# rewaifu/resselt

Hardware: AMD Instinct MI355X
Metric: output megapixels/sec, RealESRGAN-x4plus 1080p→4K, 1/2/4/8 MI355X (higher is better)
Workload: dtype fp16; 1 GPU; RealESRGAN-x4plus (RRDBNet nf64 nb23 gc32 x4), 1x3x1080x1920 fp32 frame per GPU -> 1x3x4320x7680, residual-dense-block convolutions (92 % of the MACs) in ONE fp16 product on hi planes, conv_first / upsampling / HR / last convolutions in three bf16 products on split planes, trunk convolution in three fp16 products; f32 accumulate, synthetic uniform(+-1/sqrt(fan_in)) weights; precision=auto -> mixed, io=fp32 [N,C,H,W] tensors in and out, tile_parallel=single tile

## Files before the change

include/resselt_amd.h:

```cpp
#ifndef RESSELT_AMD_H
#define RESSELT_AMD_H

#include <stdint.h>

#ifdef __cplusplus
extern "C" {
#endif

#define RSA_VERSION 400

#define RSA_OK 0
#define RSA_E_ARG (-1)
#define RSA_E_UNSUPPORTED (-2)
#define RSA_E_ALIGN (-3)
#define RSA_E_FP16_RANGE (-5)
#define RSA_E_INTERNAL (-4)

enum rsa_act {
  RSA_ACT_NONE = 0,
  RSA_ACT_LRELU = 1,
  RSA_ACT_MISH = 2,
  RSA_ACT_SILU = 3,
  RSA_ACT_GELU = 4,
  RSA_ACT_SPAB_GATE = 5,
// ... 57 lines not shown
  int32_t tile_order;
  int32_t lo8_flags;
  int32_t reserved_lo8;
  int64_t lo8_batch_stride;
} rsa_conv_params;
#define RSA_LO8_RES1 1
#define RSA_LO8_RES2 2
#define RSA_LO8_OUT 4

int rsa_conv2d(const rsa_conv_params* p, void* stream);
int rsa_conv2d_list(const rsa_conv_params* list, int32_t n, void* stream);

int rsa_conv2d_pair(const rsa_conv_params* a, const rsa_conv_params* b, void* stream);
int rsa_conv_pair_fusable(const rsa_conv_params* a, const rsa_conv_params* b);

int rsa_check_status(void);

int rsa_check_finite(const void* data, int32_t dtype, int64_t count, void* stream);

int64_t rsa_packed_weight_bytes(int32_t cout, int32_t cin_planes, int32_t ksize, int32_t products);
int64_t rsa_packed_weight_bytes_layout(int32_t cout, int32_t cin_planes, int32_t ksize, int32_t products, int32_t layout);

int rsa_conv_cout_tiles(int32_t cout);

int rsa_conv_weight_layout(const rsa_conv_params* p);
int rsa_pack_weights(const float* w_oihw, int32_t cout, int32_t cin, int32_t cin_planes, int32_t ksize, int32_t products, int32_t layout,
                     int32_t fmt, void* out, void* stream);

const char* rsa_conv_kernel_name(const rsa_conv_params* p);

int rsa_debug_ring_aborts(void);
int rsa_debug_set_ring_spin_limit(int32_t polls);
int rsa_debug_set_ring(int32_t mode);
int rsa_debug_set_pair(int32_t mode);

int rsa_nchw_to_planes(const void* x, int32_t dtype, int32_t batch, int32_t C, int32_t H, int32_t W, int32_t src_h, int32_t src_w,
                       int32_t unshuffle, const float* mean, float scale, void* out_hi, void* out_lo, int64_t out_plane_stride,
                       int64_t out_batch_stride, int32_t out_fmt, void* stream);

int rsa_planes_to_nchw(const void* hi, const void* lo, int64_t plane_stride, int64_t batch_stride, int32_t batch,
                       int32_t C, int32_t H, int32_t W, int32_t fmt, float* out, void* stream);

typedef struct rsa_dysample_params {
  int32_t batch;
  int32_t H, W;
  int32_t C;
  int32_t groups;
  int32_t scale;
  int32_t out_ch;
  const float* x_f32;
  const float* offscope;
  const float* init_pos;
  const float* end_w;
  const float* end_b;
  void* out_nchw;
  int32_t out_dtype;
} rsa_dysample_params;

int rsa_dysample(const rsa_dysample_params* p, void* stream);

typedef struct rsa_layernorm_params {
  int32_t batch;
  int32_t H, W;
  int32_t C;
  float eps;
  const float* x_f32;
// ... 716 lines not shown
```

resselt_amd/csrc/capi.hip:

```cpp
#include <hip/hip_runtime.h>
#include <stdint.h>
#include <stdio.h>
#include <string.h>

#include <type_traits>

#include "common.h"
#include "resselt_amd.h"

namespace rsa {

static thread_local char g_err[256] = "";

int set_error(int code, const char* msg) {
  if (code > 0)
    snprintf(g_err, sizeof(g_err), "%s (hipError %d: %s)", msg, code, hipGetErrorString((hipError_t)code));
  else
    snprintf(g_err, sizeof(g_err), "%s", msg);
  return code;
}

typedef __attribute__((ext_vector_type(8))) __bf16 bf16x8;

template <typename T>
// ... 218 lines not shown
  if (word == nullptr) return rsa::set_error(RSA_E_INTERNAL, "check_finite: no host-visible status word (pinned allocation failed)");
  const int64_t vecs = count / (dtype == RSA_F32 ? 4 : 8);
  const unsigned grid = rsa::grid_for(vecs > 0 ? vecs : 1, 256 * 4);
  if (dtype == RSA_F32)
    hipLaunchKernelGGL(rsa::check_finite_kernel<float>, dim3(grid), dim3(256), 0, (hipStream_t)stream, (const float*)data, count, word);
  else if (dtype == RSA_F16)
    hipLaunchKernelGGL(rsa::check_finite_kernel<_Float16>, dim3(grid), dim3(256), 0, (hipStream_t)stream, (const _Float16*)data, count, word);
  else if (dtype == RSA_BF16)
    hipLaunchKernelGGL(rsa::check_finite_kernel<__bf16>, dim3(grid), dim3(256), 0, (hipStream_t)stream, (const __bf16*)data, count, word);
  else
    return rsa::set_error(RSA_E_ARG, "check_finite: dtype must be RSA_F32, RSA_F16 or RSA_BF16");
  const int rc = (int)hipGetLastError();
  return rc ? rsa::set_error(rc, "check_finite: launch failed") : RSA_OK;
}

int rsa_conv_cout_tiles(int32_t cout) { return rsa::conv_nct(cout); }

int rsa_conv_weight_layout(const rsa_conv_params* p) {
  if (p == nullptr) return rsa::set_error(RSA_E_ARG, "rsa_conv_weight_layout: null params");
  return rsa::conv_weight_layout(*p);
}

const char* rsa_conv_kernel_name(const rsa_conv_params* p) { return p == nullptr ? "" : rsa::conv_kernel_name(*p); }

int rsa_debug_ring_aborts(void) { return (int)rsa::conv_ring_aborts(); }

int rsa_check_status(void) { return rsa::conv_check_status(); }

int rsa_debug_set_ring_spin_limit(int32_t polls) {
  rsa::conv_set_ring_spin_limit(polls);
  return RSA_OK;
}

int rsa_debug_set_ring(int32_t mode) {
  rsa::conv_ring_override(mode);
  return RSA_OK;
}

int64_t rsa_packed_weight_bytes(int32_t cout, int32_t cin_planes, int32_t ksize, int32_t products) {
  if (cout < 1 || cin_planes < 1 || (ksize != 1 && ksize != 3) || (products != 1 && products != 3)) return RSA_E_ARG;
  const int64_t ct = (cout + 15) / 16;
  const int64_t chunks = (cin_planes + 3) / 4;
  const int64_t nhl = products == 3 ? 2 : 1;
  return chunks * ksize * ksize * ct * nhl * 64 * 16;
}

int rsa_nchw_to_planes(const void* x, int32_t dtype, int32_t batch, int32_t C, int32_t H, int32_t W, int32_t src_h, int32_t src_w,
                       int32_t unshuffle, const float* mean, float scale, void* out_hi, void* out_lo, int64_t out_plane_stride,
                       int64_t out_batch_stride, int32_t out_fmt, void* stream) {
  if (out_fmt != RSA_PF_BF16 && out_fmt != RSA_PF_F16) return rsa::set_error(RSA_E_ARG, "nchw_to_planes: out_fmt must be an rsa_plane_fmt");
  if (unshuffle < 1) return rsa::set_error(RSA_E_ARG, "nchw_to_planes: unshuffle must be >= 1");
  if (x == nullptr || out_hi == nullptr || batch < 1 || C < 1 || H < 1 || W < 1) return rsa::set_error(RSA_E_ARG, "nchw_to_planes: bad argument");
  {
    const int64_t fh = (int64_t)H * unshuffle, fw = (int64_t)W * unshuffle;
    if (src_h < 1 || src_w < 1 || src_h > fh || src_w > fw || fh - src_h >= src_h || fw - src_w >= src_w)
      return rsa::set_error(RSA_E_ARG, "nchw_to_planes: source size must satisfy src <= plane size * unshuffle < 2*src (reflect padding)");
  }
  if (dtype < RSA_F32 || dtype > RSA_U8) return rsa::set_error(RSA_E_ARG, "nchw_to_planes: bad dtype");
  if (((uintptr_t)out_hi | (uintptr_t)out_lo) & 15) return rsa::set_error(RSA_E_ALIGN, "nchw_to_planes: outputs must be 16-byte aligned");
  const int64_t total = (int64_t)batch * ((C * unshuffle * unshuffle + 7) / 8) * H * W;
  hipLaunchKernelGGL(rsa::nchw_to_planes_kernel, dim3(rsa::grid_for(total, 256)), dim3(256), 0, (hipStream_t)stream, x, dtype, batch, C, H, W,
                     src_h, src_w, unshuffle, mean, scale, out_hi, out_lo, out_plane_stride, out_batch_stride, out_fmt);
  const int rc = (int)hipGetLastError();
  return rc ? rsa::set_error(rc, "nchw_to_planes: launch failed") : RSA_OK;
}

// ... 31 lines not shown
```

resselt_amd/csrc/common.h:

```cpp
#pragma once
#include <hip/hip_runtime.h>
#include <stdint.h>

#include "resselt_amd.h"

namespace rsa {

int set_error(int code, const char* msg);

int conv_launch(const rsa_conv_params& p, hipStream_t stream);
int conv_validate(const rsa_conv_params& p);
int conv_nct(int cout);
const char* conv_kernel_name(const rsa_conv_params& p);

enum { RSA_WL_TAPS = 0, RSA_WL_PAIRS = 1, RSA_WL_HALFPAIRS = 2, RSA_WL_UPPHASE = 3 };

bool conv_ring_enabled();
void conv_ring_override(int v);
inline bool conv_ring_eligible(const rsa_conv_params& p) {
  const int ct = (p.cout + 15) / 16;
  if (p.ksize != 3 || p.cin_planes < 2 || (p.cin_planes & 1)) return false;
  const bool whole = (p.cin_planes & 3) == 0;
  if (p.products == 1 && p.in_fmt != RSA_PF_F16) return false;
  if (p.in_fmt == RSA_PF_F16 && p.upsample2x) return false;
  if (p.out_nchw != nullptr) return !p.upsample2x && (ct == 3 || (ct <= 2 && whole && p.products == 3 && p.in_fmt == RSA_PF_BF16));
  if (whole) return ct == 2 || ct == 4 || (ct == 3 && !p.upsample2x);
  return ct == 3 && !p.upsample2x;
}
bool conv_ring_xres_enabled();
inline bool conv_ring_xres_eligible(const rsa_conv_params& p) {
  return p.ksize == 3 && p.products == 1 && p.in_fmt == RSA_PF_F16 && !p.upsample2x && p.cout == 64 && p.cin_planes >= 8 && (p.cin_planes & 3) == 0 &&
         p.out_nchw == nullptr && p.out_f32 == nullptr && p.res1 == nullptr && p.res2 == nullptr && p.out_hi != nullptr && p.out_lo != nullptr &&
         p.out_fmt == RSA_PF_F16 && p.res_fmt == RSA_PF_F16 && p.res1_hi != nullptr && p.res1_lo != nullptr && p.res1_hi == p.in_hi &&
         p.res_plane_stride == p.in_plane_stride && p.res_batch_stride == p.in_batch_stride && (p.res2_hi == nullptr || p.res2_lo != nullptr) &&
         (p.act == RSA_ACT_NONE || (p.act == RSA_ACT_LRELU && p.act_param >= 0.f && p.act_param <= 1.f)) &&
         (p.lo8_flags == 0 || (p.lo8_flags | RSA_LO8_OUT) == (RSA_LO8_RES1 | RSA_LO8_OUT | (p.res2_hi != nullptr ? RSA_LO8_RES2 : 0)));
}
inline bool conv_ring_em1_eligible(const rsa_conv_params& p) {
  return p.products == 1 && p.in_fmt == RSA_PF_F16 && p.out_fmt == RSA_PF_F16 && p.out_nchw == nullptr && p.out_f32 == nullptr && p.out_hi != nullptr &&
         p.out_lo == nullptr && p.res1 == nullptr && p.res2 == nullptr && p.res1_hi == nullptr && p.res2_hi == nullptr && (p.cout & 15) == 0 &&
         (p.act == RSA_ACT_NONE || (p.act == RSA_ACT_LRELU && p.act_param >= 0.f && p.act_param <= 1.f));
}
inline bool conv_ring_span_eligible(const rsa_conv_params& p) {
  const bool gate = p.act == RSA_ACT_SPAB_GATE;
  return p.ksize == 3 && p.products == 1 && p.in_fmt == RSA_PF_F16 && p.out_fmt == RSA_PF_F16 && !p.upsample2x && p.cout == 48 && (p.cin_planes & 3) != 0 &&
         p.cin_planes <= 6 && p.out_nchw == nullptr && p.out_f32 == nullptr && p.out_hi != nullptr && p.res1 == nullptr && p.res2 == nullptr && p.res2_hi == nullptr &&
         (gate ? (p.res1_hi != nullptr && p.res_fmt == RSA_PF_F16) : p.res1_hi == nullptr) &&
         (gate || p.act == RSA_ACT_MISH || p.act == RSA_ACT_SILU || p.act == RSA_ACT_NONE || (p.act == RSA_ACT_LRELU && p.act_param >= 0.f && p.act_param <= 1.f));
}
bool conv_up2_enabled();
inline bool conv_ring_up2_eligible(const rsa_conv_params& p) {
  return p.ksize == 3 && p.products == 3 && p.in_fmt == RSA_PF_BF16 && p.out_fmt == RSA_PF_BF16 && p.upsample2x && p.cin_planes == 8 && p.cout == 64 && !(p.H & 1) && !(p.W & 1) && p.out_hi != nullptr &&
         p.out_lo != nullptr && p.out_f32 == nullptr && p.out_nchw == nullptr && p.res1 == nullptr && p.res2 == nullptr && p.res1_hi == nullptr &&
         p.res2_hi == nullptr && (p.act == RSA_ACT_NONE || (p.act == RSA_ACT_LRELU && p.act_param >= 0.f && p.act_param <= 1.f));
}
bool conv_pair_enabled();
void conv_pair_override(int v);
inline bool conv_pair_eligible(const rsa_conv_params& a, const rsa_conv_params& b) {
  return a.ksize == 3 && b.ksize == 3 && !a.upsample2x && !b.upsample2x && a.cout == 32 && b.cout == 32 && conv_ring_em1_eligible(a) && conv_ring_em1_eligible(b) &&
         a.w_layout == RSA_WL_PAIRS && b.w_layout == RSA_WL_PAIRS && a.cin_planes >= 4 && (a.cin_planes & 3) == 0 && b.cin_planes == a.cin_planes + 4 &&
         a.batch == b.batch && a.H == b.H && a.W == b.W && a.in_hi == b.in_hi && a.in_plane_stride == b.in_plane_stride && a.in_batch_stride == b.in_batch_stride &&
         a.out_hi == a.in_hi && a.out_plane_off == a.cin_planes && a.out_plane_stride == a.in_plane_stride && a.out_batch_stride == a.in_batch_stride &&
// ... 26 lines not shown
```

resselt_amd/csrc/conv_inst_ring1.hip:

```cpp
#include "conv_ring.h"

namespace rsa {
int conv_launch_ring2(const rsa_conv_params& p, hipStream_t stream);
int conv_launch_ring3(const rsa_conv_params& p, hipStream_t stream);
int conv_launch_ring1_f16(const rsa_conv_params& p, hipStream_t stream);
int conv_launch_ring2_f16(const rsa_conv_params& p, hipStream_t stream);
int conv_launch_ring3_f16(const rsa_conv_params& p, hipStream_t stream);

unsigned int conv_ring2_aborts();
unsigned int conv_ring3_aborts();
unsigned int conv_ring_up2_aborts();
unsigned int conv_ring1h_aborts();
unsigned int conv_ring2h_aborts();
unsigned int conv_ring3h_aborts();
unsigned int conv_ring3hx_aborts();
unsigned int conv_ring3hs_aborts();

int conv_launch_ring(const rsa_conv_params& p, hipStream_t stream) {
  if (p.w_layout == RSA_WL_UPPHASE) return conv_launch_ring_up2(p, stream);
  const int ct = (p.cout + 15) >> 4;
  if (p.in_fmt == RSA_PF_F16) return ct == 2 ? conv_launch_ring2_f16(p, stream) : ct == 3 ? conv_launch_ring3_f16(p, stream) : conv_launch_ring1_f16(p, stream);
  if (ct <= 2) return conv_launch_ring2(p, stream);
  if (ct == 3) return conv_launch_ring3(p, stream);
  return p.upsample2x ? launch_ring<1, 1, 0>(p, stream) : launch_ring<1, 0, 0>(p, stream);
}

unsigned int conv_ring_aborts() {
  return ring_aborts_this_unit() + conv_ring2_aborts() + conv_ring3_aborts() + conv_ring_up2_aborts() + conv_ring1h_aborts() + conv_ring2h_aborts() + conv_ring3h_aborts() +
         conv_ring3hx_aborts() + conv_ring3hs_aborts() + conv_ring_pair_aborts();
}
}

#ifdef RSA_RING_DEBUG
namespace rsa {
int conv_ring2_set_dbg(unsigned v);
int conv_ring3_set_dbg(unsigned v);
int conv_ring1h_set_dbg(unsigned v);
int conv_ring2h_set_dbg(unsigned v);
int conv_ring3h_set_dbg(unsigned v);
int conv_ring3hx_set_dbg(unsigned v);
int conv_ringpair_set_dbg(unsigned v);
int conv_ring3hs_set_dbg(unsigned v);
}
extern "C" int rsa_debug_ring_flags(unsigned v) {
  if (hipMemcpyToSymbol(HIP_SYMBOL(rsa::g_ring_dbg), &v, sizeof(v)) != hipSuccess) return -1;
  return rsa::conv_ring2_set_dbg(v) | rsa::conv_ring3_set_dbg(v) | rsa::conv_ring1h_set_dbg(v) | rsa::conv_ring2h_set_dbg(v) | rsa::conv_ring3h_set_dbg(v) | rsa::conv_ring3hx_set_dbg(v) | rsa::conv_ringpair_set_dbg(v) | rsa::conv_ring3hs_set_dbg(v);
}
#endif
```

resselt_amd/csrc/conv_inst_ring1h.hip:

```cpp
#include "conv_ring.h"

namespace rsa {
int conv_launch_ring1_f16(const rsa_conv_params& p, hipStream_t stream) {
  if (p.products == 1 && conv_ring_xres_enabled() && conv_ring_xres_eligible(p)) {
    if (p.lo8_flags == 0) return launch_ring<1, 0, 0, 0, RSA_PF_F16, 1, 1>(p, stream);
    return (p.lo8_flags & RSA_LO8_OUT) ? launch_ring<1, 0, 0, 0, RSA_PF_F16, 1, 4>(p, stream) : launch_ring<1, 0, 0, 0, RSA_PF_F16, 1, 5>(p, stream);
  }
  return p.products == 1 ? launch_ring<1, 0, 0, 0, RSA_PF_F16, 1>(p, stream) : launch_ring<1, 0, 0, 0, RSA_PF_F16, 3>(p, stream);
}
unsigned int conv_ring1h_aborts() { return ring_aborts_this_unit(); }
#ifdef RSA_RING_DEBUG
int conv_ring1h_set_dbg(unsigned v) { return hipMemcpyToSymbol(HIP_SYMBOL(g_ring_dbg), &v, sizeof(v)) == hipSuccess ? 0 : -1; }
#endif
}
```

resselt_amd/csrc/conv_mfma.hip:

```cpp
#include <hip/hip_runtime.h>
#include <stdint.h>
#include <stdlib.h>

#include <stdio.h>

#include <atomic>
#include <mutex>

#include "common.h"
#include "resselt_amd.h"

namespace rsa {

int gemm_k1_launch(const rsa_conv_params& p, hipStream_t stream);
int conv_launch_k3p3u0(const rsa_conv_params& p, int nct, hipStream_t stream);
int conv_launch_k3p3u1(const rsa_conv_params& p, int nct, hipStream_t stream);
int conv_launch_k3p1u0(const rsa_conv_params& p, int nct, hipStream_t stream);
int conv_launch_k3p1u1(const rsa_conv_params& p, int nct, hipStream_t stream);
int conv_launch_k3p1u0_f16(const rsa_conv_params& p, int nct, hipStream_t stream);
int conv_launch_k3p1u1_f16(const rsa_conv_params& p, int nct, hipStream_t stream);
int conv_launch_k1p1_f16(const rsa_conv_params& p, int nct, hipStream_t stream);
int conv_launch_k3p3u0_f16(const rsa_conv_params& p, int nct, hipStream_t stream);
int conv_launch_k1p3_f16(const rsa_conv_params& p, int nct, hipStream_t stream);
int conv_launch_k1p3(const rsa_conv_params& p, int nct, hipStream_t stream);
// ... 38 lines not shown
  char msg[200];
  if (n != 0) {
    snprintf(msg, sizeof(msg), "ring schedule: %u hand-off(s) between loader and compute waves timed out; the affected launches produced wrong pixels", n);
    return set_error(RSA_E_INTERNAL, msg);
  }
  if (r != 0) {
    snprintf(msg, sizeof(msg), "fp16 range: %u block(s) of a checked tensor hold non-finite values (an activation left the fp16 range of a one-product layer, or the "
                               "input was not finite); run the model with precision 'bf16x3'", r);
    return set_error(RSA_E_FP16_RANGE, msg);
  }
  return RSA_OK;
}
static bool conv_failure_pending() {
  unsigned int* host = g_fail_host.load(std::memory_order_acquire);
  return host != nullptr && __atomic_load_n(host, __ATOMIC_ACQUIRE) != 0;
}

static std::atomic<int> g_ring_override{-1};
void conv_ring_override(int v) { g_ring_override.store(v < 0 ? -1 : (v ? 1 : 0)); }
bool conv_up2_enabled() {
  static const bool on = [] {
    const char* e = getenv("RSA_CONV_UP2");
    return !(e != nullptr && e[0] == '0');
  }();
  return on;
}
bool conv_ring_xres_enabled() {
  static const bool on = [] {
    const char* e = getenv("RSA_RING_XRES");
    return !(e != nullptr && e[0] == '0');
  }();
  return on;
}
bool conv_ring_enabled() {
  static const bool on = [] {
    const char* e = getenv("RSA_CONV_RING");
    return e == nullptr || e[0] != '0';
  }();
  const int o = g_ring_override.load(std::memory_order_relaxed);
  return o < 0 ? on : o != 0;
}

const char* conv_kernel_name(const rsa_conv_params& p) {
  if (p.w_layout == RSA_WL_UPPHASE) return "rsa::conv_ring_up2 (x2 upsampling as four 2x2 phases)";
  if (p.w_layout != RSA_WL_TAPS) {
    const int ct = (p.cout + 15) >> 4;
    if (p.products == 1) {
      if (ct == 3 && conv_ring_xres_enabled() && conv_ring_span_eligible(p)) return "rsa::conv_ring<3,0,0,HM,f16,1,XRES 3> (SPAN-family 48-channel layer, one fp16 product, weights resident in LDS, direct epilogue)";
      if (ct == 4 && conv_ring_xres_enabled() && conv_ring_xres_eligible(p)) return "rsa::conv_ring<1,0,0,0,f16,1,XRES> (conv5 of a dense block, one fp16 product, residual hi halves from the ring)";
      return ct == 2 ? "rsa::conv_ring<2,0,0,0,f16,1> (Cout<=32, one fp16 product)" : ct == 3 ? (p.out_nchw != nullptr ? "rsa::conv_ring<3,0,1,HM,f16,1> (Cout 33..48, final store, one fp16 product)" : "rsa::conv_ring<3,0,0,HM,f16,1> (Cout 33..48, one fp16 product)") : "rsa::conv_ring<1,0,0,0,f16,1> (Cout 49..64, one fp16 product)";
    }
    if (p.in_fmt == RSA_PF_F16)
      return ct == 2 ? "rsa::conv_ring<2,0,0,0,f16,3> (Cout<=32, three fp16 products)" : ct == 3 ? (p.out_nchw != nullptr ? "rsa::conv_ring<3,0,1,HM,f16,3> (Cout 33..48, final store, three fp16 products)" : "rsa::conv_ring<3,0,0,HM,f16,3> (Cout 33..48, three fp16 products)") : "rsa::conv_ring<1,0,0,0,f16,3> (Cout 49..64, three fp16 products)";
    if (ct <= 2 && p.out_nchw != nullptr) return "rsa::conv_ring<2,0,1> (Cout<=32, final store)";
    return ct == 2 ? "rsa::conv_ring<2,UP,0> (Cout<=32)" : ct == 3 ? (p.out_nchw != nullptr ? "rsa::conv_ring<3,0,1,HM> (Cout 33..48, final store)" : "rsa::conv_ring<3,0,0,HM> (Cout 33..48)") : "rsa::conv_ring<1,UP,0> (Cout 49..64)";
  }
  if (p.ksize == 1 && p.cout >= 96 && p.out_nchw == nullptr) return "rsa::gemm_k1_kernel";
  if (p.ksize == 3 && p.products == 3 && conv_nct(p.cout) == 2 && p.cout <= 32) return "rsa::conv_kernel_pp";
  return p.out_nchw != nullptr ? "rsa::conv_kernel<..., OUTK=1> (final store)" : "rsa::conv_kernel";
}

int conv_nct(int cout) {
  const int ct = (cout + 15) / 16;
  if (ct <= 4) return ct;
  const int w4 = ((ct + 3) / 4) * 4 - ct;
  const int w3 = ((ct + 2) / 3) * 3 - ct;
  return (w3 < w4) ? 3 : 4;
}

int conv_validate(const rsa_conv_params& p) {
  if (p.batch < 1 || p.H < 1 || p.W < 1 || p.cin_planes < 1 || p.cout < 1) return set_error(RSA_E_ARG, "conv: bad geometry");
  if (p.ksize != 1 && p.ksize != 3) return set_error(RSA_E_UNSUPPORTED, "conv: ksize must be 1 or 3");
  if (p.products != 1 && p.products != 3) return set_error(RSA_E_UNSUPPORTED, "conv: products must be 1 or 3");
  if ((unsigned)p.in_fmt > RSA_PF_F16 || (unsigned)p.out_fmt > RSA_PF_F16 || (unsigned)p.res_fmt > RSA_PF_F16 || (unsigned)p.tile_order > 1u)
    return set_error(RSA_E_ARG, "conv: in_fmt / out_fmt / res_fmt must be an rsa_plane_fmt, tile_order 0 or 1");
  if (conv_failure_pending()) return set_error(RSA_E_INTERNAL, "conv: an earlier ring-schedule launch reported a failed hand-off; call rsa_check_status()");
  if (p.upsample2x && (p.ksize != 3 || (p.H & 1) || (p.W & 1))) return set_error(RSA_E_UNSUPPORTED, "conv: upsample2x needs k3 and even H, W");
  if (p.in_hi == nullptr || p.w_packed == nullptr) return set_error(RSA_E_ARG, "conv: null input/weights");
  if (p.products == 3 && p.in_lo == nullptr) return set_error(RSA_E_ARG, "conv: products=3 needs in_lo");
  if (p.act == RSA_ACT_SPAB_GATE && p.res1 == nullptr && p.res1_hi == nullptr) return set_error(RSA_E_ARG, "conv: SPAB gate needs res1");
  if ((p.res1 != nullptr && p.res1_hi != nullptr) || (p.res2 != nullptr && p.res2_hi != nullptr))
// ... 77 lines not shown
```

resselt_amd/engine/lib.py:

```python

from __future__ import annotations

import ctypes as C
import os
from typing import Optional

_LIB_NAME = 'libresselt_amd.so'
_lib: Optional[C.CDLL] = None

ACT_NONE, ACT_LRELU, ACT_MISH, ACT_SILU, ACT_GELU, ACT_SPAB_GATE, ACT_PRELU = range(7)
F32, F16, BF16, U8 = range(4)
LO8_RES1, LO8_RES2, LO8_OUT = 1, 2, 4
PF_BF16, PF_F16 = range(2)
E_INTERNAL = -4


class ConvParams(C.Structure):

    _fields_ = [
        ('batch', C.c_int32),
        ('H', C.c_int32),
        ('W', C.c_int32),
        ('ksize', C.c_int32),
        ('upsample2x', C.c_int32),
# ... 735 lines not shown
        ('in_', C.c_void_p),
        ('weight', C.c_void_p),
        ('bias', C.c_void_p),
        ('out', C.c_void_p),
    ]


class EsaApplyParams(C.Structure):

    _fields_ = (
        [(k, C.c_int32) for k in ('batch', 'H', 'W', 'C', 'f', 'Hc', 'Wc', 'fmt')]
        + [(k, C.c_void_p) for k in ('x', 'c1', 'c3', 'wf', 'bf', 'w4', 'b4', 'out')]
        + _plane_fields('out')
    )


EXPORTS = (
    'rsa_version',
    'rsa_last_error_string',
    'rsa_conv2d',
    'rsa_conv2d_list',
    'rsa_conv_cout_tiles',
    'rsa_packed_weight_bytes',
    'rsa_packed_weight_bytes_layout',
    'rsa_conv_weight_layout',
    'rsa_pack_weights',
    'rsa_conv_kernel_name',
    'rsa_check_status',
    'rsa_check_finite',
    'rsa_debug_ring_aborts',
    'rsa_debug_set_ring_spin_limit',
    'rsa_debug_set_ring',
    'rsa_debug_set_pair',
    'rsa_conv2d_pair',
    'rsa_conv_pair_fusable',
    'rsa_nchw_to_planes',
    'rsa_planes_to_nchw',
    'rsa_dysample',
    'rsa_layernorm',
    'rsa_window_attention',
    'rsa_swin_attn_block',
    'rsa_swin_mlp_block',
    'rsa_swin_block',
    'rsa_rect_attention',
    'rsa_channel_attn_workspace_bytes',
    'rsa_channel_attention_weights',
    'rsa_dwconv3x3',
    'rsa_plane_stats',
    'rsa_plane_stats_fmt',
    'rsa_channel_gate_workspace_bytes',
    'rsa_channel_gate',
    'rsa_aim_combine',
    'rsa_gated_add',
    'rsa_dwconv5x5',
    'rsa_rmsnorm',
    'rsa_unshuffle_pool',
    'rsa_gated_shuffle_mul',
    'rsa_image_u8_to_nchw',
    'rsa_nchw_to_image_u8',
    'rsa_plk_packed_weight_bytes',
    'rsa_plk_conv',
    'rsa_group_norm_workspace_bytes',
    'rsa_group_norm_stats',
    'rsa_group_norm_apply',
    'rsa_ea_gate',
    'rsa_resample_packed_weight_bytes',
# ... 56 lines not shown
    path = lib_path()
    if not os.path.exists(path):
        raise RuntimeError(
            f'{_LIB_NAME} not found at {path}: build it with `python -c "import __graft_entry__ as g; g.build()"` '
            '(hipcc --offload-arch=gfx950). resselt_amd has no CPU fallback.'
        )
    _warn_if_stale(path)
    lib = C.CDLL(path)
    for name in EXPORTS:
        if not hasattr(lib, name):
            raise RuntimeError(f'{path} does not export {name}; rebuild the library')
    lib.rsa_version.restype = C.c_int
    lib.rsa_last_error_string.restype = C.c_char_p
    lib.rsa_conv2d.argtypes = [C.POINTER(ConvParams), C.c_void_p]
    lib.rsa_conv2d.restype = C.c_int
    lib.rsa_conv2d_list.argtypes = [C.POINTER(ConvParams), C.c_int32, C.c_void_p]
    lib.rsa_conv2d_list.restype = C.c_int
    lib.rsa_conv_cout_tiles.argtypes = [C.c_int32]
    lib.rsa_conv_cout_tiles.restype = C.c_int
    lib.rsa_packed_weight_bytes.argtypes = [C.c_int32] * 4
    lib.rsa_packed_weight_bytes.restype = C.c_int64
    lib.rsa_packed_weight_bytes_layout.argtypes = [C.c_int32] * 5
    lib.rsa_packed_weight_bytes_layout.restype = C.c_int64
    lib.rsa_conv_weight_layout.argtypes = [C.POINTER(ConvParams)]
    lib.rsa_conv_weight_layout.restype = C.c_int
    lib.rsa_pack_weights.argtypes = [C.c_void_p, C.c_int32, C.c_int32, C.c_int32, C.c_int32, C.c_int32, C.c_int32, C.c_int32, C.c_void_p, C.c_void_p]
    lib.rsa_pack_weights.restype = C.c_int
    lib.rsa_conv_kernel_name.argtypes = [C.POINTER(ConvParams)]
    lib.rsa_conv_kernel_name.restype = C.c_char_p
    lib.rsa_debug_ring_aborts.argtypes = []
    lib.rsa_debug_ring_aborts.restype = C.c_int
    lib.rsa_debug_set_ring.argtypes = [C.c_int32]
    lib.rsa_debug_set_ring.restype = C.c_int
    lib.rsa_debug_set_pair.argtypes = [C.c_int32]
    lib.rsa_debug_set_pair.restype = C.c_int
    lib.rsa_conv2d_pair.argtypes = [C.POINTER(ConvParams), C.POINTER(ConvParams), C.c_void_p]
    lib.rsa_conv2d_pair.restype = C.c_int
    lib.rsa_conv_pair_fusable.argtypes = [C.POINTER(ConvParams), C.POINTER(ConvParams)]
    lib.rsa_conv_pair_fusable.restype = C.c_int
    lib.rsa_debug_set_ring_spin_limit.argtypes = [C.c_int32]
    lib.rsa_debug_set_ring_spin_limit.restype = C.c_int
    lib.rsa_check_finite.argtypes = [C.c_void_p, C.c_int32, C.c_int64, C.c_void_p]
    lib.rsa_check_finite.restype = C.c_int
    lib.rsa_check_status.argtypes = []
    lib.rsa_check_status.restype = C.c_int
    lib.rsa_nchw_to_planes.argtypes = [
        C.c_void_p, C.c_int32, C.c_int32, C.c_int32, C.c_int32, C.c_int32, C.c_int32, C.c_int32, C.c_int32, C.c_void_p, C.c_float,
        C.c_void_p, C.c_void_p, C.c_int64, C.c_int64, C.c_int32, C.c_void_p,
    ]
    lib.rsa_nchw_to_planes.restype = C.c_int
    lib.rsa_planes_to_nchw.argtypes = [
        C.c_void_p, C.c_void_p, C.c_int64, C.c_int64, C.c_int32, C.c_int32, C.c_int32, C.c_int32, C.c_int32, C.c_void_p, C.c_void_p,
    ]
    lib.rsa_planes_to_nchw.restype = C.c_int
    lib.rsa_dysample.argtypes = [C.POINTER(DySampleParams), C.c_void_p]
    lib.rsa_dysample.restype = C.c_int
    lib.rsa_layernorm.argtypes = [C.POINTER(LayerNormParams), C.c_void_p]
    lib.rsa_layernorm.restype = C.c_int
    lib.rsa_window_attention.argtypes = [C.POINTER(WindowAttnParams), C.c_void_p]
    lib.rsa_window_attention.restype = C.c_int
    lib.rsa_swin_attn_block.argtypes = [C.POINTER(SwinAttnBlockParams), C.c_void_p]
    lib.rsa_swin_attn_block.restype = C.c_int
    lib.rsa_swin_mlp_block.argtypes = [C.POINTER(SwinMlpBlockParams), C.c_void_p]
    lib.rsa_swin_mlp_block.restype = C.c_int
    lib.rsa_swin_block.argtypes = [C.POINTER(SwinBlockParams), C.c_void_p]
    lib.rsa_swin_block.restype = C.c_int
# ... 98 lines not shown
def conv2d_list(params: 'C.Array[ConvParams] | list[ConvParams]', stream: int) -> None:
    lib = load()
    if isinstance(params, list):
        arr = (ConvParams * len(params))(*params)
    else:
        arr = params
    check(lib.rsa_conv2d_list(arr, len(arr), C.c_void_p(stream)), 'rsa_conv2d_list')


def conv_kernel_name(p: ConvParams) -> str:
    return load().rsa_conv_kernel_name(C.byref(p)).decode()


def ring_aborts() -> int:
    return int(load().rsa_debug_ring_aborts())


def check_status(what: str = 'forward') -> None:
    check(load().rsa_check_status(), f'{what}: rsa_check_status')


def conv2d_pair(a: ConvParams, b: ConvParams, stream: int) -> None:
    check(load().rsa_conv2d_pair(C.byref(a), C.byref(b), C.c_void_p(stream)), 'rsa_conv2d_pair')


def conv_pair_fusable(a: ConvParams, b: ConvParams) -> bool:
    return bool(load().rsa_conv_pair_fusable(C.byref(a), C.byref(b)))


def set_pair_fusion(mode: int) -> None:
    load().rsa_debug_set_pair(int(mode))


def set_ring_spin_limit(polls: int) -> None:
    load().rsa_debug_set_ring_spin_limit(int(polls))


def cout_tiles(cout: int) -> int:
    return int(load().rsa_conv_cout_tiles(cout))
```

Measured before the change: 376.4 output megapixels/s.

## Add conv5 ring kernel with two 4-wave workgroups per CU and no loader wave

Adds a specialized kernel for the conv5 layer of each residual dense block (Cout 64, one fp16 product, residual fused). Compute waves issue their own LDS ring fills and stream weights from global memory through a small register pipeline, replacing the dedicated loader wave. The launch uses two workgroups per CU so each CU holds two independent rings. It is on by default unless RSA_RING_XRES starts with '2'. The aim is better latency hiding and occupancy, at the cost of more register pressure and more complex ring synchronisation.

Measured after the change: 315.8 output megapixels/s, median of 2. 16.1% lower.

```diff
diff --git a/include/resselt_amd.h b/include/resselt_amd.h
--- a/include/resselt_amd.h
+++ b/include/resselt_amd.h
@@ -113,6 +113,7 @@
 int rsa_debug_ring_aborts(void);
 int rsa_debug_set_ring_spin_limit(int32_t polls);
 int rsa_debug_set_ring(int32_t mode);
+int rsa_debug_set_conv5_form(int32_t mode);
 int rsa_debug_set_pair(int32_t mode);
 
 int rsa_nchw_to_planes(const void* x, int32_t dtype, int32_t batch, int32_t C, int32_t H, int32_t W, int32_t src_h, int32_t src_w,
diff --git a/resselt_amd/csrc/capi.hip b/resselt_amd/csrc/capi.hip
--- a/resselt_amd/csrc/capi.hip
+++ b/resselt_amd/csrc/capi.hip
@@ -274,6 +274,11 @@
   return RSA_OK;
 }
 
+int rsa_debug_set_conv5_form(int32_t mode) {
+  rsa::conv_c5_form_override(mode);
+  return RSA_OK;
+}
+
 int rsa_debug_set_ring(int32_t mode) {
   rsa::conv_ring_override(mode);
   return RSA_OK;
diff --git a/resselt_amd/csrc/common.h b/resselt_amd/csrc/common.h
--- a/resselt_amd/csrc/common.h
+++ b/resselt_amd/csrc/common.h
@@ -28,6 +28,8 @@
   return ct == 3 && !p.upsample2x;
 }
 bool conv_ring_xres_enabled();
+int conv_c5_form();
+void conv_c5_form_override(int v);
 inline bool conv_ring_xres_eligible(const rsa_conv_params& p) {
   return p.ksize == 3 && p.products == 1 && p.in_fmt == RSA_PF_F16 && !p.upsample2x && p.cout == 64 && p.cin_planes >= 8 && (p.cin_planes & 3) == 0 &&
          p.out_nchw == nullptr && p.out_f32 == nullptr && p.res1 == nullptr && p.res2 == nullptr && p.out_hi != nullptr && p.out_lo != nullptr &&
diff --git a/resselt_amd/csrc/conv_inst_ring1.hip b/resselt_amd/csrc/conv_inst_ring1.hip
--- a/resselt_amd/csrc/conv_inst_ring1.hip
+++ b/resselt_amd/csrc/conv_inst_ring1.hip
@@ -11,6 +11,7 @@
 unsigned int conv_ring3_aborts();
 unsigned int conv_ring_up2_aborts();
 unsigned int conv_ring1h_aborts();
+unsigned int conv_ring1hx_aborts();
 unsigned int conv_ring2h_aborts();
 unsigned int conv_ring3h_aborts();
 unsigned int conv_ring3hx_aborts();
@@ -27,7 +28,7 @@
 
 unsigned int conv_ring_aborts() {
   return ring_aborts_this_unit() + conv_ring2_aborts() + conv_ring3_aborts() + conv_ring_up2_aborts() + conv_ring1h_aborts() + conv_ring2h_aborts() + conv_ring3h_aborts() +
-         conv_ring3hx_aborts() + conv_ring3hs_aborts() + conv_ring_pair_aborts();
+         conv_ring3hx_aborts() + conv_ring3hs_aborts() + conv_ring_pair_aborts() + conv_ring1hx_aborts();
 }
 }
 
diff --git a/resselt_amd/csrc/conv_inst_ring1h.hip b/resselt_amd/csrc/conv_inst_ring1h.hip
--- a/resselt_amd/csrc/conv_inst_ring1h.hip
+++ b/resselt_amd/csrc/conv_inst_ring1h.hip
@@ -1,8 +1,10 @@
 #include "conv_ring.h"
 
 namespace rsa {
+int conv_launch_ring_c5(const rsa_conv_params& p, hipStream_t stream);
 int conv_launch_ring1_f16(const rsa_conv_params& p, hipStream_t stream) {
   if (p.products == 1 && conv_ring_xres_enabled() && conv_ring_xres_eligible(p)) {
+    if (conv_c5_form() == 1) return conv_launch_ring_c5(p, stream);
     if (p.lo8_flags == 0) return launch_ring<1, 0, 0, 0, RSA_PF_F16, 1, 1>(p, stream);
     return (p.lo8_flags & RSA_LO8_OUT) ? launch_ring<1, 0, 0, 0, RSA_PF_F16, 1, 4>(p, stream) : launch_ring<1, 0, 0, 0, RSA_PF_F16, 1, 5>(p, stream);
   }
diff --git a/resselt_amd/csrc/conv_inst_ring1hx.hip b/resselt_amd/csrc/conv_inst_ring1hx.hip
--- /dev/null
+++ b/resselt_amd/csrc/conv_inst_ring1hx.hip
@@ -0,0 +1,9 @@
+#include "conv_ring_c5.h"
+
+namespace rsa {
+int conv_launch_ring_c5(const rsa_conv_params& p, hipStream_t stream) {
+  if (p.lo8_flags == 0) return launch_ring_c5<1>(p, stream);
+  return (p.lo8_flags & RSA_LO8_OUT) ? launch_ring_c5<4>(p, stream) : launch_ring_c5<5>(p, stream);
+}
+unsigned int conv_ring1hx_aborts() { return ring_aborts_this_unit(); }
+}
diff --git a/resselt_amd/csrc/conv_mfma.hip b/resselt_amd/csrc/conv_mfma.hip
--- a/resselt_amd/csrc/conv_mfma.hip
+++ b/resselt_amd/csrc/conv_mfma.hip
@@ -94,6 +94,16 @@
   }();
   return on;
 }
+static std::atomic<int> g_c5_form_override{-1};
+void conv_c5_form_override(int v) { g_c5_form_override.store(v < 0 ? -1 : (v ? 1 : 0)); }
+int conv_c5_form() {
+  static const int env = [] {
+    const char* e = getenv("RSA_RING_XRES");
+    return (e != nullptr && e[0] == '2') ? 0 : 1;
+  }();
+  const int o = g_c5_form_override.load(std::memory_order_relaxed);
+  return o < 0 ? env : o;
+}
 bool conv_ring_enabled() {
   static const bool on = [] {
     const char* e = getenv("RSA_CONV_RING");
@@ -109,6 +119,8 @@
     const int ct = (p.cout + 15) >> 4;
     if (p.products == 1) {
       if (ct == 3 && conv_ring_xres_enabled() && conv_ring_span_eligible(p)) return "rsa::conv_ring<3,0,0,HM,f16,1,XRES 3> (SPAN-family 48-channel layer, one fp16 product, weights resident in LDS, direct epilogue)";
+      if (ct == 4 && conv_ring_xres_enabled() && conv_ring_xres_eligible(p) && conv_c5_form() == 1)
+        return "rsa::conv_ring_c5<XRES> (conv5 of a dense block, one fp16 product, two 4-wave workgroups per CU, no loader wave, residual hi halves from the ring)";
       if (ct == 4 && conv_ring_xres_enabled() && conv_ring_xres_eligible(p)) return "rsa::conv_ring<1,0,0,0,f16,1,XRES> (conv5 of a dense block, one fp16 product, residual hi halves from the ring)";
       return ct == 2 ? "rsa::conv_ring<2,0,0,0,f16,1> (Cout<=32, one fp16 product)" : ct == 3 ? (p.out_nchw != nullptr ? "rsa::conv_ring<3,0,1,HM,f16,1> (Cout 33..48, final store, one fp16 product)" : "rsa::conv_ring<3,0,0,HM,f16,1> (Cout 33..48, one fp16 product)") : "rsa::conv_ring<1,0,0,0,f16,1> (Cout 49..64, one fp16 product)";
     }
diff --git a/resselt_amd/csrc/conv_ring_c5.h b/resselt_amd/csrc/conv_ring_c5.h
--- /dev/null
+++ b/resselt_amd/csrc/conv_ring_c5.h
@@ -0,0 +1,302 @@
+#pragma once
+#include "conv_ring.h"
+
+namespace rsa {
+
+#ifndef RSA_C5_WD
+#define RSA_C5_WD 2
+#endif
+#ifndef RSA_C5_DEPTH
+#define RSA_C5_DEPTH 4
+#endif
+
+template <int I>
+struct IC {
+  static constexpr int value = I;
+};
+template <int B, int E, class F>
+__device__ __forceinline__ void static_for(F&& f) {
+  if constexpr (B < E) {
+    f(IC<B>{});
+    static_for<B + 1, E>(f);
+  }
+}
+
+struct C5Geo {
+  using R = RingGeoP<1>;
+  static constexpr int NSLOT = 4, NW = 4;
+  static constexpr int DPW = R::DMA_IT / NW;
+  static_assert(R::DMA_IT % NW == 0, "a fill splits evenly over the waves");
+  static constexpr int LDS_UNITS = NSLOT * R::SLOT + R::FLAG_UNITS;
+};
+
+template <int XRES>
+__global__ __launch_bounds__(C5Geo::NW * 64, 2) void conv_ring_c5(const rsa_conv_params p, const RingAux aux) {
+  static_assert(XRES == 1 || XRES == 4 || XRES == 5, "conv5 of a residual dense block only");
+  using R = C5Geo::R;
+  constexpr int TH = R::TH, TW = R::TW, IH = R::IH, IW = R::IW, PS = R::PS, SLOT = R::SLOT;
+  constexpr int NSLOT = C5Geo::NSLOT, NW = C5Geo::NW, DPW = C5Geo::DPW;
+  constexpr int NCT = 4, CTW = 4, NPT = 8, RPW = NPT / 2, KSU = 9;
+  constexpr int WD = RSA_C5_WD, DEPTH = RSA_C5_DEPTH;
+  constexpr int FMT = RSA_PF_F16;
+  constexpr int FILL_A = 2, FILL_B = 7, PUB_A = (FILL_A + WD + 1) % KSU, PUB_B = (FILL_B + WD + 1) % KSU;
+  static_assert(WD >= 1 && WD <= 3 && PUB_B == WD - 1 && PUB_B < FILL_A && PUB_A < FILL_B, "publish points");
+
+  __shared__ uint4 s_ring[C5Geo::LDS_UNITS];
+  uint32_t* const flags = (uint32_t*)&s_ring[NSLOT * SLOT];
+  uint32_t* const f_full = flags;
+  uint32_t* const f_free = flags + 8;
+  uint32_t* const f_abort = flags + 16;
+
+  const int tid = threadIdx.x;
+  const int lane = tid & 63;
+  const int wave = __builtin_amdgcn_readfirstlane(tid >> 6);
+
+  const int tiles_x = (p.W + TW - 1) / TW;
+  const int tiles_y = (p.H + TH - 1) / TH;
+  const int num_tiles = tiles_x * tiles_y * p.batch;
+  const int nhalf = p.cin_planes >> 1;
+  const int nq = nhalf >> 1;
+  const int ct_total = (p.cout + 15) >> 4;
+
+  const int NWG = (int)gridDim.x;
+  const int tile0 = (NWG % 8 == 0) ? ((int)blockIdx.x % 8) * (NWG / 8) + (int)blockIdx.x / 8 : (int)blockIdx.x;
+  if (tile0 >= num_tiles) return;
+  const int ntw = (num_tiles - tile0 + NWG - 1) / NWG;
+
+  if (tid < 4 * R::FLAG_UNITS) flags[tid] = 0;
+  __syncthreads();
+
+  const uint32_t ring_lds = (uint32_t)(uintptr_t)(__attribute__((address_space(3))) void*)s_ring;
+  const bool half_last = wave == NW - 1 && lane >= 32;
+
+  int tn = 0, y0 = 0, x0 = 0;
+  bool interior = false;
+  int64_t tile_unit = 0;
+  uint32_t kt = 0;
+
+  auto issue_fill = [&](int h) __attribute__((always_inline)) {
+    const uint32_t k = kt + (uint32_t)h;
+    const int slot = (int)(k & (NSLOT - 1));
+    ring_wait(&f_free[slot], NW * (k / NSLOT), f_abort, aux);
+    const int hh = 2 * (nq - 1 - (h >> 1)) + (h & 1);
+    const uint32_t dst = __builtin_amdgcn_readfirstlane(ring_lds + (uint32_t)slot * (SLOT * 16) + (uint32_t)(wave * DPW) * 1024u);
+    if (interior) {
+      gcptr bh = uniform_ptr((gcptr)p.in_hi + (tile_unit + (int64_t)(2 * hh) * p.in_plane_stride) * 16);
+#pragma unroll
+      for (int i = 0; i < DPW; ++i) {
+        if (i == DPW - 1 && half_last) continue;
+        int l = lane;
+        asm volatile("" : "+v"(l));
+        const int u = (wave * DPW + i) * 64 + l;
+        const int pl = (u / PS) & 1;
+        const int r = u % PS;
+        int py = r / IW, px = r - (r / IW) * IW;
+        if (r >= IH * IW) py = 0, px = 0;
+        dma16_s(dst + i * 1024, (uint32_t)(pl * (int)p.in_plane_stride + py * p.W + px) * 16u, bh);
+      }
+    } else {
+#pragma unroll
+      for (int i = 0; i < DPW; ++i) {
+        if (i == DPW - 1 && half_last) continue;
+        int l = lane;
+        asm volatile("" : "+v"(l));
+        const int u = (wave * DPW + i) * 64 + l;
+        const int pl = (u / PS) & 1;
+        const int r = u % PS;
+        int py = r / IW, px = r - (r / IW) * IW;
+        if (r >= IH * IW) py = 0, px = 0;
+        const int iy = y0 + py, ix = x0 + px;
+        const bool ok = (uint32_t)iy < (uint32_t)p.H && (uint32_t)ix < (uint32_t)p.W;
+        const int64_t off = ((int64_t)tn * p.in_batch_stride + (int64_t)(2 * hh + pl) * p.in_plane_stride + (int64_t)iy * p.W + ix) * 16;
+        dma16_v(dst + i * 1024, ok ? (gcptr)p.in_hi + off : (gcptr)&g_zero_unit[0]);
+      }
+    }
+  };
+  auto publish = [&](int h) __attribute__((always_inline)) {
+    if (lane == 0) __hip_atomic_fetch_add(&f_full[(kt + (uint32_t)h) & (NSLOT - 1)], 1u, __ATOMIC_RELAXED, __HIP_MEMORY_SCOPE_WORKGROUP);
+  };
+
+  const int wpx = wave;
+  const int li = lane & 15;
+  const int lg = lane >> 4;
+  const int hsel = lg >> 1;
+
+  const int nks = nq * KSU;
+  const __amdgpu_buffer_rsrc_t rw = __builtin_amdgcn_make_buffer_rsrc((void*)p.w_packed, 0, (uint32_t)((int64_t)nks * ct_total * 64 * 16), 0x00020000);
+  uint32_t woff[CTW];
+#pragma unroll
+  for (int c = 0; c < CTW; ++c) woff[c] = (c < ct_total) ? (uint32_t)((c * 64 + lane) * 16) : 0xFFFFFFFFu;
+  const uint32_t wstep = (uint32_t)ct_total * 64 * 16;
+  bf16x8 wq[WD + 1][CTW];
+  auto load_w = [&](int s) __attribute__((always_inline)) {
+#pragma unroll
+    for (int c = 0; c < CTW; ++c) wq[WD][c] = __builtin_bit_cast(bf16x8, __builtin_amdgcn_raw_buffer_load_b128(rw, woff[c], (uint32_t)s * wstep, 0));
+  };
+  auto shift_w = [&]() __attribute__((always_inline)) {
+#pragma unroll
+    for (int d = 0; d < WD; ++d)
+#pragma unroll
+      for (int c = 0; c < CTW; ++c) wq[d][c] = wq[d + 1][c];
+  };
+
+  f32x4 acc[NPT][CTW];
+#pragma unroll
+  for (int pt = 0; pt < NPT; ++pt)
+#pragma unroll
+    for (int ct = 0; ct < CTW; ++ct) acc[pt][ct] = (f32x4){0.f, 0.f, 0.f, 0.f};
+
+  const int lane_u = (lg & 1) * PS + (wpx * RPW) * IW + li;
+  int uA1, uA2, uB1, uB2, uS;
+
+  auto wmap = [&](int c, int koff) -> int {
+    int cc = c + koff / KSU;
+    if (cc >= nq) cc -= nq;
+    return (nq - 1 - cc) * KSU + koff % KSU;
+  };
+#pragma unroll
+  for (int d = 0; d < WD; ++d) {
+    load_w(wmap(0, d));
+    if (d + 1 < WD) {
+#pragma unroll
+      for (int e = 1; e < WD; ++e)
+#pragma unroll
+        for (int c = 0; c < CTW; ++c) wq[e][c] = wq[e + 1][c];
+    }
+  }
+
+  for (int j = 0; j < ntw; ++j, kt += (uint32_t)nhalf) {
+    {
+      int ty, tx;
+      ring_tile_coords(p.tile_order ? num_tiles - 1 - (tile0 + j * NWG) : tile0 + j * NWG, tiles_x, tiles_y, tn, ty, tx);
+      y0 = ty * TH - 1, x0 = tx * TW - 1;
+      interior = y0 >= 0 && x0 >= 0 && y0 + IH <= p.H && x0 + IW <= p.W;
+      tile_unit = (int64_t)tn * p.in_batch_stride + (int64_t)y0 * p.W + x0;
+    }
+#pragma unroll
+    for (int h = 0; h < NSLOT; ++h) issue_fill(h);
+    asm volatile("s_waitcnt vmcnt(%0)" ::"n"(2 * DPW) : "memory");
+    publish(0);
+    publish(1);
+
+    uint32_t xslots = 0;
+    for (int c = 0; c < nq; ++c) {
+      const uint32_t kc = kt + 2u * (uint32_t)c;
+      const int sA = (int)(kc & (NSLOT - 1)), sB = (int)((kc + 1) & (NSLOT - 1));
+      const uint32_t needA = NW * (kc / NSLOT + 1), needB = NW * ((kc + 1) / NSLOT + 1);
+      const bool hold = c >= nq - 2;
+      if (c == nq - 2) xslots = (uint32_t)sA << 8 | (uint32_t)sB << 12;
+      if (c == nq - 1) xslots |= (uint32_t)sA | (uint32_t)sB << 4;
+      {
+        const int bA = sA * SLOT + lane_u, bB = sB * SLOT + lane_u;
+        uA1 = bA + hsel;
+        uA2 = bA + 2 + hsel * IW;
+        uB1 = bB + hsel;
+        uB2 = bB + 2 + hsel * IW;
+        uS = (hsel ? bB : bA) + 2 * IW + 2;
+      }
+      ring_wait(&f_full[sA], needA, f_abort, aux);
+      __builtin_amdgcn_sched_barrier(0);
+      asm volatile("" ::: "memory");
+
+      constexpr int NSTEP = KSU * NPT;
+      bf16x8 rh[DEPTH + 1];
+      auto frag = [&](int i) __attribute__((always_inline)) -> int {
+        const int ks = i / NPT, pt = i % NPT;
+        const int ptoff = (pt >> 1) * IW + (pt & 1) * 16;
+        switch (ks) {
+          case 0: return uA1 + ptoff;
+          case 1: return uA1 + IW + ptoff;
+          case 2: return uA1 + 2 * IW + ptoff;
+          case 3: return uA2 + ptoff;
+          case 4: return uS + ptoff;
+          case 5: return uB1 + ptoff;
+          case 6: return uB1 + IW + ptoff;
+          case 7: return uB1 + 2 * IW + ptoff;
+          default: return uB2 + ptoff;
+        }
+      };
+#pragma unroll
+      for (int i = 0; i < DEPTH; ++i) rh[i] = *(const bf16x8*)&s_ring[frag(i)];
+      auto step = [&](auto ic) __attribute__((always_inline)) {
+        constexpr int i = decltype(ic)::value, ks = i / NPT, sp = i % NPT;
+        if constexpr (sp == 0) {
+          if constexpr (ks == PUB_B) {
+            if (c == 0) {
+              asm volatile("s_waitcnt vmcnt(%0)" ::"n"(PUB_B * CTW) : "memory");
+              publish(2);
+              publish(3);
+            } else if (2 * c + 2 < nhalf) {
+              asm volatile("s_waitcnt vmcnt(%0)" ::"n"(WD * CTW) : "memory");
+              publish(2 * c + 2);
+            }
+          }
+          if constexpr (ks == PUB_A) if (c >= 1 && 2 * c + 3 < nhalf) {
+            asm volatile("s_waitcnt vmcnt(%0)" ::"n"(WD * CTW) : "memory");
+            publish(2 * c + 3);
+          }
+          shift_w();
+          load_w(wmap(c, ks + WD));
+          if constexpr (ks == 5) {
+            asm volatile("" ::: "memory");
+            if (lane == 0 && !hold) __hip_atomic_fetch_add(&f_free[sA], 1u, __ATOMIC_RELAXED, __HIP_MEMORY_SCOPE_WORKGROUP);
+          }
+          if constexpr (ks == FILL_A) if (c >= 1 && 2 * c + 3 < nhalf) issue_fill(2 * c + 3);
+          if constexpr (ks == FILL_B) if (2 * c + 4 < nhalf) issue_fill(2 * c + 4);
+          __builtin_amdgcn_sched_barrier(0);
+        }
+        if constexpr (i + DEPTH < NSTEP) rh[(i + DEPTH) % (DEPTH + 1)] = *(const bf16x8*)&s_ring[frag(i + DEPTH)];
+#pragma unroll
+        for (int ct = 0; ct < CTW; ++ct) acc[sp][ct] = mfma16<FMT>(wq[0][ct], rh[i % (DEPTH + 1)], acc[sp][ct]);
+        if constexpr (i + DEPTH < NSTEP) __builtin_amdgcn_sched_group_barrier(0x100, 1, 0);
+        __builtin_amdgcn_sched_group_barrier(0x008, CTW, 0);
+        __builtin_amdgcn_sched_barrier(0);
+      };
+      constexpr int FIRST_B = 4 * NPT - DEPTH;
+      static_for<0, FIRST_B>(step);
+      ring_wait(&f_full[sB], needB, f_abort, aux);
+      __builtin_amdgcn_sched_barrier(0);
+      asm volatile("" ::: "memory");
+      static_for<FIRST_B, NSTEP>(step);
+      asm volatile("" ::: "memory");
+      if (lane == 0 && !hold) __hip_atomic_fetch_add(&f_free[sB], 1u, __ATOMIC_RELAXED, __HIP_MEMORY_SCOPE_WORKGROUP);
+    }
+    {
+      const int ey0 = y0 + 1, ex0 = x0 + 1;
+      if (p.res2_hi != nullptr)
+        epilogue_impl<NCT, CTW, NPT, 0, AC_LINEAR, 3, RSA_PF_F16, 1, XRES == 4 ? 1 : (XRES == 5 ? 2 : 0)>(p, acc, tn, ey0, ex0, 0, 0, wpx, li, lg, s_ring, xslots, SLOT, PS, IW);
+      else
+        epilogue_impl<NCT, CTW, NPT, 0, AC_LINEAR, 2, RSA_PF_F16, 1, XRES == 4 ? 1 : (XRES == 5 ? 2 : 0)>(p, acc, tn, ey0, ex0, 0, 0, wpx, li, lg, s_ring, xslots, SLOT, PS, IW);
+      asm volatile("s_waitcnt lgkmcnt(0)" ::: "memory");
+      if (lane == 0) {
+#pragma unroll
+        for (int q = 0; q < 4; ++q) __hip_atomic_fetch_add(&f_free[(xslots >> (4 * q)) & 15u], 1u, __ATOMIC_RELAXED, __HIP_MEMORY_SCOPE_WORKGROUP);
+      }
+    }
+#pragma unroll
+    for (int pt = 0; pt < NPT; ++pt)
+#pragma unroll
+      for (int ct = 0; ct < CTW; ++ct) acc[pt][ct] = (f32x4){0.f, 0.f, 0.f, 0.f};
+  }
+}
+
+template <int XRES>
+static int launch_ring_c5(const rsa_conv_params& p, hipStream_t stream) {
+  using R = C5Geo::R;
+  const int tiles_x = (p.W + R::TW - 1) / R::TW;
+  const int tiles_y = (p.H + R::TH - 1) / R::TH;
+  const int64_t num_tiles = (int64_t)tiles_x * tiles_y * p.batch;
+  if (num_tiles > 0x3fffffff / 2) return RSA_E_UNSUPPORTED;
+  static const int cus = [] {
+    int dev = 0;
+    hipDeviceProp_t prop;
+    if (hipGetDevice(&dev) != hipSuccess || hipGetDeviceProperties(&prop, dev) != hipSuccess) return 256;
+    return prop.multiProcessorCount;
+  }();
+  int gx = 2 * cus;
+  if (gx > num_tiles) gx = (int)num_tiles;
+  hipLaunchKernelGGL((conv_ring_c5<XRES>), dim3((unsigned)gx, 1, 1), dim3(C5Geo::NW * 64), 0, stream, p, ring_aux());
+  return (int)hipGetLastError();
+}
+
+}
diff --git a/resselt_amd/engine/lib.py b/resselt_amd/engine/lib.py
--- a/resselt_amd/engine/lib.py
+++ b/resselt_amd/engine/lib.py
@@ -791,6 +791,7 @@
     'rsa_debug_set_ring_spin_limit',
     'rsa_debug_set_ring',
     'rsa_debug_set_pair',
+    'rsa_debug_set_conv5_form',
     'rsa_conv2d_pair',
     'rsa_conv_pair_fusable',
     'rsa_nchw_to_planes',
@@ -913,6 +914,8 @@
     lib.rsa_debug_ring_aborts.restype = C.c_int
     lib.rsa_debug_set_ring.argtypes = [C.c_int32]
     lib.rsa_debug_set_ring.restype = C.c_int
+    lib.rsa_debug_set_conv5_form.argtypes = [C.c_int32]
+    lib.rsa_debug_set_conv5_form.restype = C.c_int
     lib.rsa_debug_set_pair.argtypes = [C.c_int32]
     lib.rsa_debug_set_pair.restype = C.c_int
     lib.rsa_conv2d_pair.argtypes = [C.POINTER(ConvParams), C.POINTER(ConvParams), C.c_void_p]
@@ -1077,6 +1080,10 @@
     load().rsa_debug_set_pair(int(mode))
 
 
+def set_conv5_form(mode: int) -> None:
+    load().rsa_debug_set_conv5_form(int(mode))
+
+
 def set_ring_spin_limit(polls: int) -> None:
     load().rsa_debug_set_ring_spin_limit(int(polls))
 
```
